# jason-li-831202/Vehicle-CV-ADAS

Hardware: AMD Instinct MI355X
Metric: frames/sec end-to-end (detect+lane+NMS+track) per GPU; conv MFMA util % (higher is better)
Workload: dtype fp16x3

## Files before the change

vehicle-cv-adas_amd/csrc/conv_halo_s2.hip:

```cpp
#include "kernels.h"
#include "elem16.h"
#include <stdlib.h>
#include <map>
#include <mutex>
#include <tuple>
#include <type_traits>

namespace adas {

typedef __attribute__((ext_vector_type(4))) float sf32x4_;
typedef __attribute__((ext_vector_type(4))) uint32_t su32x4_;

template <int ACT>
__device__ __forceinline__ float s2_act(float v) {
    if (ACT == ACT_SILU) return v * fast_rcp(1.0f + __expf(-v));
    if (ACT == ACT_RELU) return fmaxf(v, 0.0f);
    if (ACT == ACT_LEAKY) return fmaxf(v, 0.1f * v);
    return v;
}

struct S2Dev {
    const uint16_t* in;
    const uint16_t* wgt;
    const float* bias;
// ... 211 lines not shown
        const bool ok = plan_s2_uncached(Ho, Wo, &p);
        it = cache.emplace(key, std::make_pair(ok, p)).first;
    }
    *out = it->second.second;
    return it->second.first;
}

static bool s2p_enabled() {
    static int v = -1;
    if (v < 0) {
        const char* e = getenv("ADAS_NO_HALO_S2P");
        v = (e && e[0] == '1') ? 0 : 1;
    }
    return v == 1;
}

bool halo_s2p_applicable(const ConvArgs& a) {
    const TView &in = a.in, &out = a.out;
    if (!s2p_enabled() || a.stride != 2 || a.kh != 3 || a.kw != 3 || a.pad != 1 || a.res_mode != RES_NONE) return false;
    if (in.f32 || out.f32 || out.h != (in.h + 2 - 3) / 2 + 1 || out.w != (in.w + 2 - 3) / 2 + 1) return false;
    if ((in.c & 7) || (in.cs & 7) || (in.coff & 7) || (out.c & 127) || (out.cs & 3) || (out.coff & 3)) return false;
    if (in.c < 16 || (long)in.h * in.w * in.cs >= (1L << 30)) return false;
    if (in.c < 128) return false;
    S2Plan pl;
    if (!plan_s2(out.h, out.w, &pl) || pl.eff < 0.45) return false;
    return (long)a.n * pl.NS * pl.TPS * (out.c / 128) >= 512;
}

hipError_t launch_conv_halo_s2p(const ConvArgs& a, hipStream_t st) {
    S2Plan pl;
    if (!halo_s2p_applicable(a) || !plan_s2(a.out.h, a.out.w, &pl)) return hipErrorInvalidValue;
    S2Dev d;
    d.in = (const uint16_t*)a.in.p; d.wgt = (const uint16_t*)a.wgt; d.bias = a.bias; d.out = (uint16_t*)a.out.p;
    d.in_cs = a.in.cs; d.in_coff = a.in.coff; d.cin = a.in.c; d.H = a.in.h; d.W = a.in.w;
    d.out_cs = a.out.cs; d.out_coff = a.out.coff; d.cout = a.out.c;
    d.cin_pad = (a.in.c + 31) / 32 * 32;
    d.SW = pl.SW; d.NS = pl.NS; d.TPS = pl.TPS; d.PW = pl.PW; d.plane = pl.plane;
    d.npix4 = 4 * pl.plane * 4;
    d.Ho = a.out.h; d.Wo = a.out.w;
    d.mg_pw = pl.mg_pw; d.mg_sw = pl.mg_sw; d.mg_plane = pl.mg_plane;
    d.ntiles = a.n * pl.NS * pl.TPS;
    d.tiles8 = (d.ntiles + 7) / 8;
    d.ncb = a.out.c / 128;
    { static int xm = -1; if (xm < 0) { const char* e = getenv("ADAS_HALO_XMAP"); xm = e ? atoi(e) : 1; } d.xmap = xm; }
    const dim3 grid(8 * d.tiles8 * d.ncb);
    const size_t lds = ((size_t)4 * pl.plane * 32 + (size_t)2 * S2_WROWS * 32) * 2;
    static bool attr_done = false;
    if (!attr_done) {
#define S2_ATTR(E_, A_) (void)hipFuncSetAttribute((const void*)conv_s2p_kernel<E_, A_>, hipFuncAttributeMaxDynamicSharedMemorySize, 160 * 1024)
        S2_ATTR(Bf16, ACT_NONE); S2_ATTR(Bf16, ACT_SILU); S2_ATTR(Bf16, ACT_RELU); S2_ATTR(Bf16, ACT_LEAKY);
        S2_ATTR(Fp16, ACT_NONE); S2_ATTR(Fp16, ACT_SILU); S2_ATTR(Fp16, ACT_RELU); S2_ATTR(Fp16, ACT_LEAKY);
#undef S2_ATTR
        attr_done = true;
    }
    ADAS_DISPATCH_E16(a.prec == PREC_FP16, E, {
        if (a.act == ACT_SILU) hipLaunchKernelGGL((conv_s2p_kernel<E, ACT_SILU>), grid, dim3(S2_THR), lds, st, d);
        else if (a.act == ACT_RELU) hipLaunchKernelGGL((conv_s2p_kernel<E, ACT_RELU>), grid, dim3(S2_THR), lds, st, d);
        else if (a.act == ACT_LEAKY) hipLaunchKernelGGL((conv_s2p_kernel<E, ACT_LEAKY>), grid, dim3(S2_THR), lds, st, d);
        else hipLaunchKernelGGL((conv_s2p_kernel<E, ACT_NONE>), grid, dim3(S2_THR), lds, st, d);
    });
    return hipGetLastError();
}

struct S2XDev {
    const unsigned char* in;
    const uint16_t* wgt;
    const float* bias;
    x3s* out;
    int in_cs, in_coff, cin, H, W;
    int out_cs, out_coff, cout;
    int nck;
    int SW, NS, TPS, PW, plane;
    int npix4;
    int Ho, Wo;
    uint32_t mg_pw, mg_sw, mg_plane;
    int ntiles, tiles8, ncb, xmap;
};

template <int ACT>
__device__ __forceinline__ float s2x_act(float v) {
    if (ACT == ACT_SILU) return x3_silu(v);
    if (ACT == ACT_RELU) return fmaxf(v, 0.0f);
    if (ACT == ACT_LEAKY) return fmaxf(v, 0.1f * v);
    return v;
}

#ifdef ADAS_S2X_PROF
__device__ unsigned long long g_s2x_prof[16];
#define S2XP(i)                                     \
    if (tid == 0) {                                 \
        const unsigned long long t__ = clock64();   \
        pacc__[i] += t__ - tprev__;                 \
        tprev__ = t__;                              \
    }
#else
#define S2XP(i)
#endif

template <int ACT>
__global__ __launch_bounds__(S2_THR, 1) void conv_s2p_x3_kernel(S2XDev a) {
    Fp16::enter();
    typedef Fp16::vec8 vec8;
    constexpr int TAPS = 9, TM = 4;
    extern __shared__ __attribute__((aligned(16))) uint16_t lds[];
    uint16_t* Aw = lds;
    uint16_t* Ww = lds + (size_t)4 * a.plane * 32;

    const int tid = threadIdx.x, lane = tid & 63, wave = tid >> 6;
    const int lrow = lane & 15, kg = lane >> 4;
    const int half = wave >> 2, grp = wave & 3;
#ifdef ADAS_S2X_PROF
    unsigned long long tprev__ = clock64();
    unsigned long long pacc__[8] = {0, 0, 0, 0, 0, 0, 0, 0};
#endif
    const int xslot = blockIdx.x >> 3;
    const int xr = xslot / a.ncb;
    const int cb = xslot - xr * a.ncb;
    int tile = a.xmap ? (int)(blockIdx.x & 7) * a.tiles8 + xr : xr * 8 + (blockIdx.x & 7);
    if (tile >= a.ntiles) return;
    const int n0 = cb * 64 + half * 32;
    const int per_img = a.NS * a.TPS;
    const int img = tile / per_img;
    tile -= img * per_img;
    const int strip = tile / a.TPS, t = tile - strip * a.TPS;
    const int sx0 = strip * a.SW, p0 = t * S2_BM;
    const int y_first = (int)(((uint32_t)p0 * a.mg_sw) >> 20);
    const int wy0 = 2 * y_first - 1, wx0 = 2 * sx0 - 1;

    const unsigned char* in_img = a.in + ((size_t)img * a.H * a.W * a.in_cs + a.in_coff) * 4;
    __amdgpu_buffer_rsrc_t rsrc = __builtin_amdgcn_make_buffer_rsrc((void*)in_img, 0, (a.H * a.W * a.in_cs - a.in_coff) * 4, 0x00020000);
    uint32_t goff[S2_NA];
#pragma unroll
    for (int i = 0; i < S2_NA; ++i) {
        const int e = tid + S2_THR * i;
        const int pix = e >> 2, c8 = e & 3;
        const int q = (int)(((uint32_t)pix * a.mg_plane) >> 20);
        const int pp = pix - q * a.plane;
        const int py = (int)(((uint32_t)pp * a.mg_pw) >> 20), px = pp - py * a.PW;
        const int iy = wy0 + 2 * py + (q >> 1), ix = wx0 + 2 * px + (q & 1);
        const bool ok = e < a.npix4 && (unsigned)iy < (unsigned)a.H && (unsigned)ix < (unsigned)a.W;
        goff[i] = ok ? (uint32_t)((iy * a.W + ix) * a.in_cs * 4 + c8 * 32) : 0x80000000u;
    }
    const uint16_t* wb0 = a.wgt + (size_t)(2 * cb) * a.nck * S2_WROWS * 32;
    const uint16_t* wb1 = wb0 + (size_t)a.nck * S2_WROWS * 32;
    const int gsw[4] = {0, 2, 3, 1};
    const int wdst0 = ((tid & ~3) + ((tid & 3) ^ gsw[(tid >> 4) & 3])) * 8;
    const int wrd = (half * S2_WROWS + lrow) * 32 + ((kg ^ gsw[(lrow >> 2) & 3]) << 3);

    int apl[TM], oy[TM], ox[TM];
#pragma unroll
    for (int j = 0; j < TM; ++j) {
        const int p = p0 + (grp * TM + j) * 16 + lrow;
        const int y = (int)(((uint32_t)p * a.mg_sw) >> 20), xs = p - y * a.SW;
        oy[j] = y;
        ox[j] = sx0 + xs;
        apl[j] = (y - y_first) * a.PW + xs;
    }

    sf32x4_ acc[4][TM];
#pragma unroll
    for (int i = 0; i < 2; ++i) {
        const float4 b = *reinterpret_cast<const float4*>(a.bias + n0 + i * 16 + kg * 4);
#pragma unroll
        for (int j = 0; j < TM; ++j) {
            acc[i][j] = sf32x4_{b.x, b.y, b.z, b.w};
            acc[i + 2][j] = sf32x4_{0.f, 0.f, 0.f, 0.f};
        }
    }

    su32x4_ ra[S2_NA], rw[S2_NW];
    auto gload = [&](int ck, auto with_w) {
        const uint32_t cofs = (uint32_t)((ck >> 1) * 128 + (ck & 1) * 16);
#pragma unroll
        for (int i = 0; i < S2_NA; ++i) ra[i] = __builtin_amdgcn_raw_buffer_load_b128(rsrc, goff[i] + cofs, 0, 0);
        if constexpr (!decltype(with_w)::value) return;
#pragma unroll
        for (int i = 0; i < S2_NW; ++i) {
            const int e = tid + S2_THR * i;
            const uint16_t* src = (e < S2_WROWS * 4 ? wb0 + (size_t)e * 8 : wb1 + (size_t)(e - S2_WROWS * 4) * 8) + (size_t)ck * S2_WROWS * 32;
            rw[i] = *reinterpret_cast<const su32x4_*>(src);
        }
    };
    const int na = (a.npix4 + S2_THR - 1) / S2_THR;
    auto lstore = [&](auto with_w) {
#pragma unroll
        for (int i = 0; i < S2_NA; ++i) {
            const int e = tid + S2_THR * i;
            if (i < na && e < a.npix4) *reinterpret_cast<su32x4_*>(Aw + (e >> 2) * 32 + (((e & 3) ^ ((e >> 3) & 2)) << 3)) = ra[i];
        }
        if constexpr (!decltype(with_w)::value) return;
#pragma unroll
        for (int i = 0; i < S2_NW; ++i) *reinterpret_cast<su32x4_*>(Ww + wdst0 + i * S2_THR * 8) = rw[i];
    };
    auto taps = [&](auto lo_c) {
        constexpr int I0 = decltype(lo_c)::value ? 2 : 0;
#pragma unroll
        for (int tap = 0; tap < TAPS; ++tap) {
            const int r = tap / 3, s = tap - r * 3;
            const int tofs = ((r & 1) * 2 + (s & 1)) * a.plane + (r >> 1) * a.PW + (s >> 1);
            vec8 wf[4], xf[TM];
#pragma unroll
            for (int i = I0; i < 4; ++i) wf[i] = *reinterpret_cast<const vec8*>(Ww + (tap * 64 + (i - I0) * 16) * 32 + wrd);
#pragma unroll
            for (int j = 0; j < TM; ++j) {
                const int pw = apl[j] + tofs;
                xf[j] = *reinterpret_cast<const vec8*>(Aw + pw * 32 + ((kg ^ ((pw >> 1) & 2)) << 3));
            }
#pragma unroll
            for (int i = I0; i < 4; ++i)
#pragma unroll
                for (int j = 0; j < TM; ++j) acc[i][j] = Fp16::mfma(wf[i], xf[j], acc[i][j]);
        }
    };

    S2XP(0)
    gload(0, std::true_type{});
    lstore(std::true_type{});
    __syncthreads();
    S2XP(1)
    for (int ck = 0; ck < a.nck; ck += 2) {
        gload(ck + 1, std::false_type{});
        taps(std::false_type{});
        S2XP(2)
        __syncthreads();
        S2XP(3)
        lstore(std::false_type{});
        __syncthreads();
        S2XP(4)
        if (ck + 2 < a.nck) gload(ck + 2, std::true_type{});
        taps(std::true_type{});
        S2XP(5)
        if (ck + 2 < a.nck) {
            __syncthreads();
            lstore(std::true_type{});
            __syncthreads();
            S2XP(6)
        }
    }

#pragma unroll
    for (int j = 0; j < TM; ++j) {
        const bool pok = oy[j] < a.Ho && ox[j] < a.Wo;
        const size_t mpix = pok ? ((size_t)img * a.Ho + oy[j]) * a.Wo + ox[j] : 0;
#pragma unroll
        for (int i = 0; i < 2; ++i) {
            float v[4];
#pragma unroll
            for (int e = 0; e < 4; ++e) v[e] = s2x_act<ACT>(acc[i][j][e] + acc[i + 2][j][e] * kX3Down);
            const int c = n0 + i * 16 + kg * 4;
            if (pok && c < a.cout) x3_store4(a.out + mpix * a.out_cs + a.out_coff + c, v);
        }
    }
#ifdef ADAS_S2X_PROF
    S2XP(7)
    if (tid == 0) {
        for (int i__ = 0; i__ < 8; ++i__) atomicAdd(&g_s2x_prof[i__], pacc__[i__]);
        atomicAdd(&g_s2x_prof[8], 1ull);
    }
#endif
}

#ifdef ADAS_S2X_PROF
extern "C" int adas_debug_s2x_prof(unsigned long long* out16, int reset) {
    static unsigned long long h[16];
    if (out16 && hipMemcpyFromSymbol(out16, HIP_SYMBOL(g_s2x_prof), sizeof(h)) != hipSuccess) return -1;
    if (reset) {
        for (int i = 0; i < 16; ++i) h[i] = 0;
        if (hipMemcpyToSymbol(HIP_SYMBOL(g_s2x_prof), h, sizeof(h)) != hipSuccess) return -1;
    }
    return 0;
}
#endif

struct S2DDev {
    const void* in;
    const void* wgt;
    const float* bias;
    void* out;
    uint32_t in_bytes, wgt_bytes, out_bytes;
    int in_cs, in_coff, cin, H, W;
    int out_cs, out_coff, cout, Ho, Wo;
    int nck;
    int SW, NS, TPS, PW, PH, plane16;
    uint32_t mg_pw, mg_sw;
    int ntiles, tiles8, ncb, xmap;
};
typedef __attribute__((address_space(3))) void* slds_vp;
typedef __attribute__((ext_vector_type(2))) float sf32x2_;
constexpr uint32_t S2D_OOB = 0xF0000000u;
constexpr int S2D_TAP = 2 * 64 * 64;
constexpr int S2D_SLAB = 9 * 64 * 64;


template <int N>
__device__ __forceinline__ void s2d_wait_vm() {
    asm volatile("s_waitcnt vmcnt(%0)" ::"n"(N) : "memory");
}
template <int ACT>
__device__ __forceinline__ sf32x2_ s2d_act2(sf32x2_ v) {
    if (ACT == ACT_RELU) return __builtin_elementwise_max(v, sf32x2_{0.0f, 0.0f});
    return sf32x2_{s2x_act<ACT>(v[0]), s2x_act<ACT>(v[1])};
}

#ifdef ADAS_S2D_PROF
__device__ unsigned long long g_s2d_prof[16];
#define S2DP(i)                                     \
    if (tid == 0) {                                 \
        const unsigned long long t__ = clock64();   \
        pacc__[i] += t__ - tprev__;                 \
        tprev__ = t__;                              \
    }
#else
#define S2DP(i)
#endif

template <int ACT, int NP>
__global__ __launch_bounds__(S2_THR, 1) void conv_s2d_x3_kernel(S2DDev a) {
    Fp16::enter();
    typedef Fp16::vec8 vec8;
    extern __shared__ __attribute__((aligned(16))) uint8_t s2d_lds[];
    const int WOFF = 4 * a.plane16 * 64;

    const int tid = threadIdx.x, lane = tid & 63;
    const int wave = __builtin_amdgcn_readfirstlane(tid >> 6);
    const int lrow = lane & 15, kg = lane >> 4;
    const int hb = wave >> 2, grp = wave & 3;
#ifdef ADAS_S2D_PROF
    unsigned long long tprev__ = clock64();
    unsigned long long pacc__[8] = {0, 0, 0, 0, 0, 0, 0, 0};
    unsigned long long nitem__ = 0;
#endif
    __amdgpu_buffer_rsrc_t rin = __builtin_amdgcn_make_buffer_rsrc((void*)a.in, 0, a.in_bytes, 0x00020000);
    __amdgpu_buffer_rsrc_t rwg = __builtin_amdgcn_make_buffer_rsrc((void*)a.wgt, 0, a.wgt_bytes, 0x00020000);
    __amdgpu_buffer_rsrc_t rout = __builtin_amdgcn_make_buffer_rsrc((void*)a.out, 0, a.out_bytes, 0x00020000);
    const int gsw[4] = {0, 2, 3, 1};
    const uint32_t wlane = (uint32_t)((lane >> 2) * 64 + (((lane & 3) ^ gsw[(lane >> 4) & 3]) << 4));
    const uint32_t wrd = (uint32_t)(WOFF + hb * 4096 + lrow * 64 + ((kg ^ gsw[(lrow >> 2) & 3]) << 4));
    const uint32_t ch_lane = (uint32_t)((hb * 4 + (kg >> 1)) * 32 + (kg & 1) * 16);

    struct Item {
        int img, cb, sx0, p0, y_first;
    };
    const int nvb = 8 * a.tiles8 * a.ncb, per_img = a.NS * a.TPS;
    auto decode = [&](int v, Item& it) -> bool {
        if (v >= nvb) return false;
        const int xslot = v >> 3, xr = xslot / a.ncb;
        int tile = a.xmap ? (v & 7) * a.tiles8 + xr : xr * 8 + (v & 7);
        if (tile >= a.ntiles) return false;
        it.cb = xslot - xr * a.ncb;
        it.img = tile / per_img;
        tile -= it.img * per_img;
        const int strip = tile / a.TPS, t = tile - strip * a.TPS;
        it.sx0 = strip * a.SW;
        it.p0 = t * S2_BM;
        it.y_first = (int)(((uint32_t)it.p0 * a.mg_sw) >> 20);
        return true;
    };
    int vb = blockIdx.x;
    const int vstep = gridDim.x;
    Item cur, nxt;
    if (!decode(vb, cur)) return;
    bool has_next = decode(vb + vstep, nxt);

    const int npieces = a.plane16 >> 4;
    int pj[3];
#pragma unroll
    for (int n = 0; n < NP; ++n) pj[n] = wave + 8 * n < npieces ? wave + 8 * n : wave % npieces;
    auto src_offset = [&](const Item& it, int q, int n) {
        int lz;
        asm volatile("v_mov_b32 %0, %1" : "=v"(lz) : "v"(lane));
        const int px = pj[n] * 16 + (lz >> 2);
        const int grpk = (lz & 3) ^ ((px >> 1) & 2);
        const int py = (int)(((uint32_t)px * a.mg_pw) >> 20), pxx = px - py * a.PW;
        const int iy = 2 * it.y_first - 1 + 2 * py + (q >> 1), ix = 2 * it.sx0 - 1 + 2 * pxx + (q & 1);
        const bool ok = py < a.PH && (unsigned)iy < (unsigned)a.H && (unsigned)ix < (unsigned)a.W;
        const uint32_t off = ((uint32_t)((it.img * a.H + iy) * a.W + ix) * (uint32_t)a.in_cs + (uint32_t)a.in_coff) * 4u + (uint32_t)(grpk << 5);
        const uint32_t m = 0u - (uint32_t)ok;
        return (off & m) | (S2D_OOB & ~m);
    };
    uint32_t gsrc[4][3];
    auto wgt_base = [&](int cb) { return (uint32_t)(((2 * cb + hb) * a.nck) * S2D_SLAB + grp * 1024); };
    auto issue_tile = [&](int tap, uint32_t wsrc, uint32_t woob) {
        __builtin_amdgcn_raw_ptr_buffer_load_lds(rwg, (slds_vp)(s2d_lds + WOFF + tap * S2D_TAP + wave * 1024), 16, wlane | woob, wsrc + (uint32_t)tap * 4096u, 0, 0);
    };

    uint32_t apl[4], po[4];
    auto set_output = [&](const Item& it) {
#pragma unroll
        for (int j = 0; j < 4; ++j) {
            const int p = it.p0 + (grp * 4 + j) * 16 + lrow;
            const int y = (int)(((uint32_t)p * a.mg_sw) >> 20), xs = p - y * a.SW;
            apl[j] = (uint32_t)((y - it.y_first) * a.PW + xs);
            const int ox = it.sx0 + xs;
            po[j] = (y < a.Ho && ox < a.Wo) ? (uint32_t)((it.img * a.Ho + y) * a.Wo + ox) : S2D_OOB;
        }
    };
    const uint32_t kg16 = (uint32_t)(kg << 4);
    auto frag_addr = [&](int j, int t) {
        const int r = t / 3, sx = t % 3;
        const uint32_t pw = apl[j] + (uint32_t)((r >> 1) * a.PW + (sx >> 1));
        return ((uint32_t)(((r & 1) * 2 + (sx & 1)) * a.plane16) + pw) * 64u + (kg16 ^ ((pw << 3) & 0x20u));
    };
    sf32x4_ acc[4][4];
    float4 bias4[2];
#pragma unroll
    for (int i = 0; i < 2; ++i) bias4[i] = *reinterpret_cast<const float4*>(a.bias + cur.cb * 64 + hb * 32 + i * 16 + kg * 4);
    auto reset_acc = [&]() {
#pragma unroll
        for (int i = 0; i < 2; ++i) {
#pragma unroll
            for (int j = 0; j < 4; ++j) {
                acc[i][j] = sf32x4_{bias4[i].x, bias4[i].y, bias4[i].z, bias4[i].w};
                acc[i + 2][j] = sf32x4_{0.f, 0.f, 0.f, 0.f};
            }
        }
    };

    struct Pend {
        uint32_t wsrc, woob;
        bool last;
    };
    auto issue_piece = [&](auto q_c, auto g_c, auto lo_c, auto k_c, const Pend& pd) {
        constexpr int q = decltype(q_c)::value, g = decltype(g_c)::value, k = decltype(k_c)::value;
        constexpr bool pislo = decltype(lo_c)::value;
        if constexpr (k < NP) {
            __builtin_amdgcn_raw_ptr_buffer_load_lds(rin, (slds_vp)(s2d_lds + (q * a.plane16 + pj[k] * 16) * 64), 16, gsrc[q][k], 0, 0, 0);
            if (pd.last) gsrc[q][k] = has_next ? src_offset(nxt, q, k) : S2D_OOB;
            else gsrc[q][k] += pislo ? 16u : 112u;
        } else {
            constexpr int tl[4][4] = {{4, 4, 4, 4}, {1, 7, 7, 7}, {3, 5, 5, 5}, {0, 2, 6, 8}};
            issue_tile(tl[g][k - NP], pd.wsrc, pd.woob);
        }
    };

    const uint32_t wcur = wgt_base(cur.cb);
#pragma unroll
    for (int q = 0; q < 4; ++q)
#pragma unroll
        for (int n = 0; n < NP; ++n) gsrc[q][n] = src_offset(cur, q, n);
    {
        const Pend p0{wcur, 0u, false};
        auto slot = [&](auto q_c, auto g_c) {
            constexpr int g = decltype(g_c)::value;
            constexpr int nt = g == 0 ? 1 : 2;
            issue_piece(q_c, g_c, std::true_type{}, std::integral_constant<int, 0>{}, p0);
            issue_piece(q_c, g_c, std::true_type{}, std::integral_constant<int, 1>{}, p0);
            if constexpr (NP > 2) issue_piece(q_c, g_c, std::true_type{}, std::integral_constant<int, 2>{}, p0);
            issue_piece(q_c, g_c, std::true_type{}, std::integral_constant<int, NP>{}, p0);
            if constexpr (nt > 1) issue_piece(q_c, g_c, std::true_type{}, std::integral_constant<int, NP + 1>{}, p0);
        };
        slot(std::integral_constant<int, 3>{}, std::integral_constant<int, 0>{});
        slot(std::integral_constant<int, 1>{}, std::integral_constant<int, 1>{});
        slot(std::integral_constant<int, 2>{}, std::integral_constant<int, 2>{});
    }
    set_output(cur);
    reset_acc();
    s2d_wait_vm<0>();
    __builtin_amdgcn_s_barrier();
    S2DP(0)

    for (;;) {
        const uint32_t wnext = wcur;
        const uint32_t woob_next = has_next ? 0u : S2D_OOB;

        auto half_chunk = [&](auto lo_c, const int ck) {
            constexpr bool islo = decltype(lo_c)::value;
            constexpr int I0 = islo ? 2 : 0, NI = islo ? 2 : 4;
#pragma unroll
            for (int j = 0; j < 4; ++j) asm volatile("" : "+v"(apl[j]));
            const bool to_next_item = ck + 1 >= a.nck;
            const Pend pprev{wcur + (uint32_t)ck * S2D_SLAB, 0u, ck - 1 == a.nck - 2};
            const Pend pthis{to_next_item ? wnext : wcur + (uint32_t)(ck + 1) * S2D_SLAB, to_next_item ? woob_next : 0u, ck == a.nck - 2};
            auto tap = [&](auto t_c, auto pq_c, auto pg_c, auto pl_c, auto k0_c, auto k1_c, const Pend& pd) {
                constexpr int t = decltype(t_c)::value, K0 = decltype(k0_c)::value, K1 = decltype(k1_c)::value;
                vec8 wf[4], xf[4];
#pragma unroll
                for (int i = I0; i < 4; ++i) wf[i] = *reinterpret_cast<const vec8*>(s2d_lds + wrd + t * S2D_TAP + (i - I0) * 1024);
#pragma unroll
                for (int j = 0; j < 4; ++j) xf[j] = *reinterpret_cast<const vec8*>(s2d_lds + frag_addr(j, t));
                auto block = [&](auto b_c) {
                    constexpr int b = decltype(b_c)::value;
                    if constexpr (b < NI) {
#pragma unroll
                        for (int j = 0; j < 4; ++j) acc[I0 + b][j] = Fp16::mfma(wf[I0 + b], xf[j], acc[I0 + b][j]);
                        constexpr int ka = K0 + (K1 - K0) * b / NI, kb = K0 + (K1 - K0) * (b + 1) / NI;
                        if constexpr (kb > ka) issue_piece(pq_c, pg_c, pl_c, std::integral_constant<int, ka>{}, pd);
                        if constexpr (kb > ka + 1) issue_piece(pq_c, pg_c, pl_c, std::integral_constant<int, ka + 1>{}, pd);
                        if constexpr (kb > ka + 2) issue_piece(pq_c, pg_c, pl_c, std::integral_constant<int, ka + 2>{}, pd);
                        static_assert(kb <= ka + 3, "at most three pieces between two MFMA blocks");
                    }
                };
                block(std::integral_constant<int, 0>{}); block(std::integral_constant<int, 1>{});
                block(std::integral_constant<int, 2>{}); block(std::integral_constant<int, 3>{});
            };
            auto close = [&](auto g_c) {
                constexpr int g = decltype(g_c)::value;
                constexpr int allow = 2 * NP + (islo ? (g == 0 ? 0 : (g == 1 ? 1 : (g == 2 ? 3 : 4))) : (g == 0 ? 6 : (g == 1 ? 4 : 0)));
                __builtin_amdgcn_sched_barrier(0);
                S2DP(islo ? 2 : 1)
                s2d_wait_vm<allow>();
                S2DP(3)
                __builtin_amdgcn_s_barrier();
                __builtin_amdgcn_sched_barrier(0);
                S2DP(4)
            };
            using std::integral_constant;
            typedef integral_constant<bool, !islo> PrevL;
            typedef integral_constant<bool, islo> ThisL;
            constexpr int P3 = NP + (!islo ? 4 : 0), P0 = NP + (islo ? 1 : 0), P1 = NP + (islo ? 2 : 0), P2 = NP + (islo ? 2 : 0);
            tap(integral_constant<int, 4>{}, integral_constant<int, 0>{}, integral_constant<int, 3>{}, PrevL{}, integral_constant<int, 0>{}, integral_constant<int, P3>{}, pprev);
            close(integral_constant<int, 0>{});
            tap(integral_constant<int, 1>{}, integral_constant<int, 3>{}, integral_constant<int, 0>{}, ThisL{}, integral_constant<int, 0>{}, integral_constant<int, P0 / 2>{}, pthis);
            tap(integral_constant<int, 7>{}, integral_constant<int, 3>{}, integral_constant<int, 0>{}, ThisL{}, integral_constant<int, P0 / 2>{}, integral_constant<int, P0>{}, pthis);
            close(integral_constant<int, 1>{});
            tap(integral_constant<int, 3>{}, integral_constant<int, 1>{}, integral_constant<int, 1>{}, ThisL{}, integral_constant<int, 0>{}, integral_constant<int, P1 / 2>{}, pthis);
            tap(integral_constant<int, 5>{}, integral_constant<int, 1>{}, integral_constant<int, 1>{}, ThisL{}, integral_constant<int, P1 / 2>{}, integral_constant<int, P1>{}, pthis);
            close(integral_constant<int, 2>{});
            tap(integral_constant<int, 0>{}, integral_constant<int, 2>{}, integral_constant<int, 2>{}, ThisL{}, integral_constant<int, 0>{}, integral_constant<int, P2 / 4>{}, pthis);
            tap(integral_constant<int, 2>{}, integral_constant<int, 2>{}, integral_constant<int, 2>{}, ThisL{}, integral_constant<int, P2 / 4>{}, integral_constant<int, P2 / 2>{}, pthis);
            tap(integral_constant<int, 6>{}, integral_constant<int, 2>{}, integral_constant<int, 2>{}, ThisL{}, integral_constant<int, P2 / 2>{}, integral_constant<int, 3 * P2 / 4>{}, pthis);
            tap(integral_constant<int, 8>{}, integral_constant<int, 2>{}, integral_constant<int, 2>{}, ThisL{}, integral_constant<int, 3 * P2 / 4>{}, integral_constant<int, P2>{}, pthis);
            close(integral_constant<int, 3>{});
        };
        for (int ck = 0; ck < a.nck; ck += 2) {
            half_chunk(std::false_type{}, ck);
            half_chunk(std::true_type{}, ck + 1);
        }
        S2DP(5)

        {
            const uint32_t ch0 = (uint32_t)(cur.cb * 256) + ch_lane;
#pragma unroll
            for (int j = 0; j < 4; ++j) {
                sf32x2_ val[2][2];
                uint32_t hw[2][2];
#pragma unroll
                for (int i = 0; i < 2; ++i) {
                    val[i][0] = s2d_act2<ACT>(sf32x2_{acc[i + 2][j][0], acc[i + 2][j][1]} * kX3Down + sf32x2_{acc[i][j][0], acc[i][j][1]});
                    val[i][1] = s2d_act2<ACT>(sf32x2_{acc[i + 2][j][2], acc[i + 2][j][3]} * kX3Down + sf32x2_{acc[i][j][2], acc[i][j][3]});
                }
                __builtin_amdgcn_s_setreg((unsigned short)(1 | (6 << 6) | (1 << 11)), 0u);
#pragma unroll
                for (int i = 0; i < 2; ++i)
#pragma unroll
                    for (int h = 0; h < 2; ++h) asm volatile("v_cvt_pk_f16_f32 %0, %1, %2" : "=v"(hw[i][h]) : "v"(val[i][h][0]), "v"(val[i][h][1]));
                __builtin_amdgcn_s_setreg((unsigned short)(1 | (6 << 6) | (1 << 11)), 3u);
                const uint32_t oo = po[j] == S2D_OOB ? S2D_OOB : (po[j] * (uint32_t)a.out_cs + (uint32_t)a.out_coff) * 4u + ch0;
#pragma unroll
                for (int i = 0; i < 2; ++i) {
                    const uint32_t oi = (cur.cb * 64 + hb * 32 + i * 16 + (kg >> 1) * 8 < a.cout) ? oo + i * 64 : S2D_OOB;
                    uint32_t lw[2];
#pragma unroll
                    for (int h = 0; h < 2; ++h) {
                        const sf32x2_ d = (val[i][h] - __builtin_convertvector(__builtin_bit_cast(e_f16x2, hw[i][h]), sf32x2_)) * kX3Up;
                        lw[h] = __builtin_bit_cast(uint32_t, __builtin_convertvector(d, e_f16x2));
                    }
                    const auto s0 = __builtin_amdgcn_permlane16_swap(hw[i][0], lw[0], false, false);
                    const auto s1 = __builtin_amdgcn_permlane16_swap(hw[i][1], lw[1], false, false);
                    __builtin_amdgcn_raw_buffer_store_b128(su32x4_{s0[0], s1[0], s0[1], s1[1]}, rout, oi, 0, 0);
                }
            }
        }
        S2DP(6)
#ifdef ADAS_S2D_PROF
        ++nitem__;
#endif
        if (!has_next) break;
        cur = nxt;
        vb += vstep;
        has_next = decode(vb + vstep, nxt);
        set_output(cur);
        reset_acc();
        S2DP(7)
    }
#ifdef ADAS_S2D_PROF
    if (tid == 0) {
        for (int i__ = 0; i__ < 8; ++i__) atomicAdd(&g_s2d_prof[i__], pacc__[i__]);
        atomicAdd(&g_s2d_prof[8], nitem__);
    }
#endif
    s2d_wait_vm<0>();
}

#ifdef ADAS_S2D_PROF
extern "C" int adas_debug_s2d_prof(unsigned long long* out16, int reset) {
    static unsigned long long h[16];
    if (out16 && hipMemcpyFromSymbol(out16, HIP_SYMBOL(g_s2d_prof), sizeof(h)) != hipSuccess) return -1;
    if (reset) {
        for (int i = 0; i < 16; ++i) h[i] = 0;
        if (hipMemcpyToSymbol(HIP_SYMBOL(g_s2d_prof), h, sizeof(h)) != hipSuccess) return -1;
    }
    return 0;
}
#endif

static bool s2x_enabled() {
    static int v = -1;
    if (v < 0) {
        const char* e = getenv("ADAS_NO_HALO_S2P_X3");
        v = (e && e[0] == '1') ? 0 : 1;
    }
    return v == 1;
}

bool halo_s2p_x3_shape_ok(int kh, int kw, int stride, int pad, int res_mode, const TView& in, const TView& out) {
    if (!s2x_enabled() || stride != 2 || kh != 3 || kw != 3 || pad != 1 || res_mode != RES_NONE) return false;
    if (in.f32 || out.f32 || out.h != (in.h + 2 - 3) / 2 + 1 || out.w != (in.w + 2 - 3) / 2 + 1) return false;
    if ((in.c & 31) || (in.cs & 7) || (in.coff & 7) || (out.c & 7) || (out.cs & 7) || (out.coff & 7)) return false;
    if ((long)in.h * in.w * in.cs * 4 >= (1L << 31)) return false;
    if (2 * out.c < (out.c + 63) / 64 * 64) return false;
    S2Plan pl;
    return plan_s2(out.h, out.w, &pl) && pl.eff >= 0.45;
}

bool halo_s2p_x3_applicable(const ConvArgs& a) {
    if (!halo_s2p_x3_shape_ok(a.kh, a.kw, a.stride, a.pad, a.res_mode, a.in, a.out)) return false;
    S2Plan pl;
    if (!plan_s2(a.out.h, a.out.w, &pl)) return false;
    static long min_items = -1;
    if (min_items < 0) { const char* e = getenv("ADAS_S2X_MIN_ITEMS"); min_items = e ? atol(e) : 96; if (min_items < 1) min_items = 96; }
    return (long)a.n * pl.NS * pl.TPS * ((a.out.c + 63) / 64) >= min_items;
}

bool s2d_x3_fits(const ConvArgs& a) {
    const TView &in = a.in, &out = a.out;
    const int n = a.n;
    static int on = -1;
    if (on < 0) { const char* e = getenv("ADAS_NO_S2D_X3"); on = (e && e[0] == '1') ? 0 : 1; }
    const size_t in_bytes = (size_t)n * in.h * in.w * in.cs * 4, out_bytes = (size_t)n * out.h * out.w * out.cs * 4;
    const int ncb = (out.c + 63) / 64, nck = 2 * (in.c / 32);
    const size_t wgt_bytes = (size_t)2 * ncb * nck * S2D_SLAB;
    return on && ncb <= 32 && in_bytes < 0x70000000ull && out_bytes < 0x70000000ull && wgt_bytes < 0x70000000ull;
}
hipError_t launch_conv_s2d_x3(const ConvArgs& a, hipStream_t st) {
    S2Plan pl;
    if (!a.wgt_h8x3 || !halo_s2p_x3_applicable(a) || !s2d_x3_fits(a) || !plan_s2(a.out.h, a.out.w, &pl)) return hipErrorInvalidValue;
    const size_t in_bytes = (size_t)a.n * a.in.h * a.in.w * a.in.cs * 4, out_bytes = (size_t)a.n * a.out.h * a.out.w * a.out.cs * 4;
    const int ncb = (a.out.c + 63) / 64, nck = 2 * (a.in.c / 32);
    const size_t wgt_bytes = (size_t)2 * ncb * nck * S2D_SLAB;
    S2DDev d;
    d.in = a.in.p; d.wgt = a.wgt_h8x3; d.bias = a.bias; d.out = a.out.p;
    d.in_bytes = (uint32_t)in_bytes; d.wgt_bytes = (uint32_t)wgt_bytes; d.out_bytes = (uint32_t)out_bytes;
    d.in_cs = a.in.cs; d.in_coff = a.in.coff; d.cin = a.in.c; d.H = a.in.h; d.W = a.in.w;
    d.out_cs = a.out.cs; d.out_coff = a.out.coff; d.cout = a.out.c; d.Ho = a.out.h; d.Wo = a.out.w;
    d.nck = nck;
    d.SW = pl.SW; d.NS = pl.NS; d.TPS = pl.TPS; d.PW = pl.PW;
    d.PH = (S2_BM + pl.SW - 1) / pl.SW + ((S2_BM % pl.SW) ? 1 : 0) + 1;
    d.plane16 = (d.PH * d.PW + 15) / 16 * 16;
    d.mg_pw = pl.mg_pw; d.mg_sw = pl.mg_sw;
    d.ntiles = a.n * pl.NS * pl.TPS;
    d.tiles8 = (d.ntiles + 7) / 8;
    d.ncb = ncb;
    { static int xm = -1; if (xm < 0) { const char* e = getenv("ADAS_HALO_XMAP"); xm = e ? atoi(e) : 1; } d.xmap = xm; }
    const size_t lds = (size_t)4 * d.plane16 * 64 + 9 * S2D_TAP;
    if (lds > 160 * 1024) return hipErrorInvalidValue;
    const int nvb = 8 * d.tiles8 * d.ncb;
    static int rounds = -1;
    if (rounds < 0) { const char* e = getenv("ADAS_S2D_ROUNDS"); rounds = e ? atoi(e) : 16; if (rounds < 1 || rounds > 16) rounds = 16; }
    const int gmax = 8 * d.ncb * (32 / d.ncb) * rounds;
    const dim3 grid(nvb > gmax ? gmax : nvb);
    static bool attr_done = false;
    if (!attr_done) {
#define S2D_ATTR(A_) (void)hipFuncSetAttribute((const void*)conv_s2d_x3_kernel<A_, 2>, hipFuncAttributeMaxDynamicSharedMemorySize, 160 * 1024); \
                     (void)hipFuncSetAttribute((const void*)conv_s2d_x3_kernel<A_, 3>, hipFuncAttributeMaxDynamicSharedMemorySize, 160 * 1024)
        S2D_ATTR(ACT_NONE); S2D_ATTR(ACT_SILU); S2D_ATTR(ACT_RELU); S2D_ATTR(ACT_LEAKY);
#undef S2D_ATTR
        attr_done = true;
    }
    const bool np3 = d.plane16 > 256;
#define S2D_GO(A_) do { if (np3) hipLaunchKernelGGL((conv_s2d_x3_kernel<A_, 3>), grid, dim3(S2_THR), lds, st, d); \
                        else hipLaunchKernelGGL((conv_s2d_x3_kernel<A_, 2>), grid, dim3(S2_THR), lds, st, d); } while (0)
    if (a.act == ACT_SILU) S2D_GO(ACT_SILU);
    else if (a.act == ACT_RELU) S2D_GO(ACT_RELU);
    else if (a.act == ACT_LEAKY) S2D_GO(ACT_LEAKY);
    else S2D_GO(ACT_NONE);
#undef S2D_GO
    return hipGetLastError();
}

hipError_t launch_conv_s2p_x3(const ConvArgs& a, hipStream_t st) {
    S2Plan pl;
    if (!a.wgt_h8x3 || !halo_s2p_x3_applicable(a) || !plan_s2(a.out.h, a.out.w, &pl)) return hipErrorInvalidValue;
    S2XDev d;
    d.in = (const unsigned char*)a.in.p; d.wgt = (const uint16_t*)a.wgt_h8x3; d.bias = a.bias; d.out = (x3s*)a.out.p;
    d.in_cs = a.in.cs; d.in_coff = a.in.coff; d.cin = a.in.c; d.H = a.in.h; d.W = a.in.w;
    d.out_cs = a.out.cs; d.out_coff = a.out.coff; d.cout = a.out.c;
    d.nck = 2 * (a.in.c / 32);
    d.SW = pl.SW; d.NS = pl.NS; d.TPS = pl.TPS; d.PW = pl.PW; d.plane = pl.plane;
    d.npix4 = 4 * pl.plane * 4;
    d.Ho = a.out.h; d.Wo = a.out.w;
    d.mg_pw = pl.mg_pw; d.mg_sw = pl.mg_sw; d.mg_plane = pl.mg_plane;
    d.ntiles = a.n * pl.NS * pl.TPS;
    d.tiles8 = (d.ntiles + 7) / 8;
    d.ncb = (a.out.c + 63) / 64;
    { static int xm = -1; if (xm < 0) { const char* e = getenv("ADAS_HALO_XMAP"); xm = e ? atoi(e) : 1; } d.xmap = xm; }
    const dim3 grid(8 * d.tiles8 * d.ncb);
    const size_t lds = ((size_t)4 * pl.plane * 32 + (size_t)2 * S2_WROWS * 32) * 2;
    static bool attr_done = false;
    if (!attr_done) {
#define S2X_ATTR(A_) (void)hipFuncSetAttribute((const void*)conv_s2p_x3_kernel<A_>, hipFuncAttributeMaxDynamicSharedMemorySize, 160 * 1024)
        S2X_ATTR(ACT_NONE); S2X_ATTR(ACT_SILU); S2X_ATTR(ACT_RELU); S2X_ATTR(ACT_LEAKY);
#undef S2X_ATTR
        attr_done = true;
    }
    if (a.act == ACT_SILU) hipLaunchKernelGGL((conv_s2p_x3_kernel<ACT_SILU>), grid, dim3(S2_THR), lds, st, d);
    else if (a.act == ACT_RELU) hipLaunchKernelGGL((conv_s2p_x3_kernel<ACT_RELU>), grid, dim3(S2_THR), lds, st, d);
    else if (a.act == ACT_LEAKY) hipLaunchKernelGGL((conv_s2p_x3_kernel<ACT_LEAKY>), grid, dim3(S2_THR), lds, st, d);
    else hipLaunchKernelGGL((conv_s2p_x3_kernel<ACT_NONE>), grid, dim3(S2_THR), lds, st, d);
    return hipGetLastError();
}

}
```

Baseline: 5598.

## Merge stride-2 conv load slots into three stages and precompute fragment addresses

Restructures the per-chunk load and MMA pipeline of the stride-2 fp16x3 conv from four wait groups to three: the q=3 and q=1 input-plane loads are merged into one slot, and the weight-tap order and wait counts are rebalanced. The prologue is staggered with scheduling barriers, and the initial wait no longer drains all loads. Per-row LDS fragment base addresses are precomputed per 2x2 sub-offset, and output pixel offsets are computed only in the epilogue, to cut address arithmetic in the hot loop at some register cost. The epilogue also narrows the rounding-mode switches to a subset of the packed conversions per row, which can change rounding of the high half while relying on the residual half to compensate.

```diff
diff --git a/vehicle-cv-adas_amd/csrc/conv_halo_s2.hip b/vehicle-cv-adas_amd/csrc/conv_halo_s2.hip
--- a/vehicle-cv-adas_amd/csrc/conv_halo_s2.hip
+++ b/vehicle-cv-adas_amd/csrc/conv_halo_s2.hip
@@ -537,6 +537,21 @@
     return sf32x2_{s2x_act<ACT>(v[0]), s2x_act<ACT>(v[1])};
 }
 
+__host__ __device__ constexpr int s2d_flush_first(int act, int j) { return act == ACT_SILU ? (j == 0 ? 2 : 1) : 0; }
+__host__ __device__ constexpr int s2d_flush_count(int act, int j) {
+    return act == ACT_SILU ? (j == 0 ? 2 : (j == 3 ? 0 : 3)) : (act == ACT_LEAKY ? (j == 0 ? 0 : 2) : 0);
+}
+__device__ __forceinline__ void s2d_cvt_hi_flushed(uint32_t& h0, uint32_t& h1, sf32x2_ a, sf32x2_ b) {
+    asm volatile("s_setreg_imm32_b32 hwreg(HW_REG_MODE, 6, 2), 0\n\ts_nop 1\n\tv_cvt_pk_f16_f32 %0, %2, %3\n\tv_cvt_pk_f16_f32 %1, %4, %5\n\t"
+                 "s_setreg_imm32_b32 hwreg(HW_REG_MODE, 6, 2), 3\n\ts_nop 1"
+                 : "=&v"(h0), "=&v"(h1) : "v"(a[0]), "v"(a[1]), "v"(b[0]), "v"(b[1]));
+}
+__device__ __forceinline__ void s2d_cvt_hi_flushed(uint32_t& h0, uint32_t& h1, uint32_t& h2, sf32x2_ a, sf32x2_ b, sf32x2_ c) {
+    asm volatile("s_setreg_imm32_b32 hwreg(HW_REG_MODE, 6, 2), 0\n\ts_nop 1\n\tv_cvt_pk_f16_f32 %0, %3, %4\n\tv_cvt_pk_f16_f32 %1, %5, %6\n\t"
+                 "v_cvt_pk_f16_f32 %2, %7, %8\n\ts_setreg_imm32_b32 hwreg(HW_REG_MODE, 6, 2), 3\n\ts_nop 1"
+                 : "=&v"(h0), "=&v"(h1), "=&v"(h2) : "v"(a[0]), "v"(a[1]), "v"(b[0]), "v"(b[1]), "v"(c[0]), "v"(c[1]));
+}
+
 #ifdef ADAS_S2D_PROF
 __device__ unsigned long long g_s2d_prof[16];
 #define S2DP(i)                                     \
@@ -568,9 +583,10 @@
     __amdgpu_buffer_rsrc_t rin = __builtin_amdgcn_make_buffer_rsrc((void*)a.in, 0, a.in_bytes, 0x00020000);
     __amdgpu_buffer_rsrc_t rwg = __builtin_amdgcn_make_buffer_rsrc((void*)a.wgt, 0, a.wgt_bytes, 0x00020000);
     __amdgpu_buffer_rsrc_t rout = __builtin_amdgcn_make_buffer_rsrc((void*)a.out, 0, a.out_bytes, 0x00020000);
-    const int gsw[4] = {0, 2, 3, 1};
-    const uint32_t wlane = (uint32_t)((lane >> 2) * 64 + (((lane & 3) ^ gsw[(lane >> 4) & 3]) << 4));
-    const uint32_t wrd = (uint32_t)(WOFF + hb * 4096 + lrow * 64 + ((kg ^ gsw[(lrow >> 2) & 3]) << 4));
+    auto gsw = [](int x) { return (0x78 >> (2 * x)) & 3; };
+
+    const uint32_t wlane = (uint32_t)((lane >> 2) * 64 + (((lane & 3) ^ gsw((lane >> 4) & 3)) << 4));
+    const uint32_t wrd = (uint32_t)(WOFF + hb * 4096 + lrow * 64 + ((kg ^ gsw((lrow >> 2) & 3)) << 4));
     const uint32_t ch_lane = (uint32_t)((hb * 4 + (kg >> 1)) * 32 + (kg & 1) * 16);
 
     struct Item {
@@ -619,22 +635,30 @@
         __builtin_amdgcn_raw_ptr_buffer_load_lds(rwg, (slds_vp)(s2d_lds + WOFF + tap * S2D_TAP + wave * 1024), 16, wlane | woob, wsrc + (uint32_t)tap * 4096u, 0, 0);
     };
 
-    uint32_t apl[4], po[4];
+    const uint32_t kg16 = (uint32_t)(kg << 4);
+    const uint32_t splane = (uint32_t)(a.plane16 * 64);
+    uint32_t fa[4][4];
     auto set_output = [&](const Item& it) {
 #pragma unroll
         for (int j = 0; j < 4; ++j) {
             const int p = it.p0 + (grp * 4 + j) * 16 + lrow;
             const int y = (int)(((uint32_t)p * a.mg_sw) >> 20), xs = p - y * a.SW;
-            apl[j] = (uint32_t)((y - it.y_first) * a.PW + xs);
-            const int ox = it.sx0 + xs;
-            po[j] = (y < a.Ho && ox < a.Wo) ? (uint32_t)((it.img * a.Ho + y) * a.Wo + ox) : S2D_OOB;
-        }
-    };
-    const uint32_t kg16 = (uint32_t)(kg << 4);
+            const uint32_t ap = (uint32_t)((y - it.y_first) * a.PW + xs);
+#pragma unroll
+            for (int st = 0; st < 4; ++st) {
+                const uint32_t pw = ap + (uint32_t)((st >> 1) * a.PW + (st & 1));
+                fa[j][st] = pw * 64u + (kg16 ^ ((pw << 3) & 0x20u));
+            }
+        }
+    };
+    auto out_pixel = [&](const Item& it, int j) {
+        const int p = it.p0 + (grp * 4 + j) * 16 + lrow;
+        const int y = (int)(((uint32_t)p * a.mg_sw) >> 20), ox = it.sx0 + p - y * a.SW;
+        return (y < a.Ho && ox < a.Wo) ? (uint32_t)((it.img * a.Ho + y) * a.Wo + ox) : S2D_OOB;
+    };
     auto frag_addr = [&](int j, int t) {
         const int r = t / 3, sx = t % 3;
-        const uint32_t pw = apl[j] + (uint32_t)((r >> 1) * a.PW + (sx >> 1));
-        return ((uint32_t)(((r & 1) * 2 + (sx & 1)) * a.plane16) + pw) * 64u + (kg16 ^ ((pw << 3) & 0x20u));
+        return fa[j][(r >> 1) * 2 + (sx >> 1)] + (uint32_t)((r & 1) * 2 + (sx & 1)) * splane;
     };
     sf32x4_ acc[4][4];
     float4 bias4[2];
@@ -655,42 +679,49 @@
         uint32_t wsrc, woob;
         bool last;
     };
-    auto issue_piece = [&](auto q_c, auto g_c, auto lo_c, auto k_c, const Pend& pd) {
-        constexpr int q = decltype(q_c)::value, g = decltype(g_c)::value, k = decltype(k_c)::value;
+    auto issue_piece = [&](auto s_c, auto lo_c, auto k_c, const Pend& pd) {
+        constexpr int S = decltype(s_c)::value, k = decltype(k_c)::value;
         constexpr bool pislo = decltype(lo_c)::value;
-        if constexpr (k < NP) {
-            __builtin_amdgcn_raw_ptr_buffer_load_lds(rin, (slds_vp)(s2d_lds + (q * a.plane16 + pj[k] * 16) * 64), 16, gsrc[q][k], 0, 0, 0);
-            if (pd.last) gsrc[q][k] = has_next ? src_offset(nxt, q, k) : S2D_OOB;
-            else gsrc[q][k] += pislo ? 16u : 112u;
+        constexpr int NWIN = S == 0 ? 2 * NP : NP;
+        if constexpr (k < NWIN) {
+            constexpr int q = S == 0 ? (k < NP ? 3 : 1) : (S == 1 ? 2 : 0), n = k < NP ? k : k - NP;
+            __builtin_amdgcn_raw_ptr_buffer_load_lds(rin, (slds_vp)(s2d_lds + (q * a.plane16 + pj[n] * 16) * 64), 16, gsrc[q][n], 0, 0, 0);
+            if (pd.last) gsrc[q][n] = has_next ? src_offset(nxt, q, n) : S2D_OOB;
+            else gsrc[q][n] += pislo ? 16u : 112u;
         } else {
-            constexpr int tl[4][4] = {{4, 4, 4, 4}, {1, 7, 7, 7}, {3, 5, 5, 5}, {0, 2, 6, 8}};
-            issue_tile(tl[g][k - NP], pd.wsrc, pd.woob);
-        }
-    };
+            constexpr int tl[3][4] = {{4, 1, 7, 7}, {3, 5, 5, 5}, {0, 2, 6, 8}};
+            issue_tile(tl[S][k - NWIN], pd.wsrc, pd.woob);
+        }
+    };
+    typedef std::integral_constant<int, 0> SlotA;
+    typedef std::integral_constant<int, 1> SlotB;
+    typedef std::integral_constant<int, 2> SlotC;
 
     const uint32_t wcur = wgt_base(cur.cb);
-#pragma unroll
-    for (int q = 0; q < 4; ++q)
-#pragma unroll
-        for (int n = 0; n < NP; ++n) gsrc[q][n] = src_offset(cur, q, n);
     {
         const Pend p0{wcur, 0u, false};
-        auto slot = [&](auto q_c, auto g_c) {
-            constexpr int g = decltype(g_c)::value;
-            constexpr int nt = g == 0 ? 1 : 2;
-            issue_piece(q_c, g_c, std::true_type{}, std::integral_constant<int, 0>{}, p0);
-            issue_piece(q_c, g_c, std::true_type{}, std::integral_constant<int, 1>{}, p0);
-            if constexpr (NP > 2) issue_piece(q_c, g_c, std::true_type{}, std::integral_constant<int, 2>{}, p0);
-            issue_piece(q_c, g_c, std::true_type{}, std::integral_constant<int, NP>{}, p0);
-            if constexpr (nt > 1) issue_piece(q_c, g_c, std::true_type{}, std::integral_constant<int, NP + 1>{}, p0);
-        };
-        slot(std::integral_constant<int, 3>{}, std::integral_constant<int, 0>{});
-        slot(std::integral_constant<int, 1>{}, std::integral_constant<int, 1>{});
-        slot(std::integral_constant<int, 2>{}, std::integral_constant<int, 2>{});
-    }
+#define S2D_PK(S_, K_) issue_piece(S_{}, std::true_type{}, std::integral_constant<int, K_>{}, p0)
+        S2D_PK(SlotA, 2 * NP); S2D_PK(SlotA, 2 * NP + 1); S2D_PK(SlotA, 2 * NP + 2); S2D_PK(SlotB, NP); S2D_PK(SlotB, NP + 1);
+        __builtin_amdgcn_sched_barrier(0);
+#pragma unroll
+        for (int n = 0; n < NP; ++n) gsrc[3][n] = src_offset(cur, 3, n);
+#pragma unroll
+        for (int n = 0; n < NP; ++n) gsrc[1][n] = src_offset(cur, 1, n);
+        S2D_PK(SlotA, 0); S2D_PK(SlotA, 1); S2D_PK(SlotA, 2); S2D_PK(SlotA, 3);
+        if constexpr (NP > 2) { S2D_PK(SlotA, 4); S2D_PK(SlotA, 5); }
+        __builtin_amdgcn_sched_barrier(0);
+#pragma unroll
+        for (int n = 0; n < NP; ++n) gsrc[2][n] = src_offset(cur, 2, n);
+        S2D_PK(SlotB, 0); S2D_PK(SlotB, 1);
+        if constexpr (NP > 2) S2D_PK(SlotB, 2);
+        __builtin_amdgcn_sched_barrier(0);
+#undef S2D_PK
+    }
+#pragma unroll
+    for (int n = 0; n < NP; ++n) gsrc[0][n] = src_offset(cur, 0, n);
     set_output(cur);
     reset_acc();
-    s2d_wait_vm<0>();
+    s2d_wait_vm<NP>();
     __builtin_amdgcn_s_barrier();
     S2DP(0)
 
@@ -702,11 +733,11 @@
             constexpr bool islo = decltype(lo_c)::value;
             constexpr int I0 = islo ? 2 : 0, NI = islo ? 2 : 4;
 #pragma unroll
-            for (int j = 0; j < 4; ++j) asm volatile("" : "+v"(apl[j]));
+            for (int j = 0; j < 4; ++j) asm volatile("" : "+v"(fa[j][0]), "+v"(fa[j][1]), "+v"(fa[j][2]), "+v"(fa[j][3]));
             const bool to_next_item = ck + 1 >= a.nck;
             const Pend pprev{wcur + (uint32_t)ck * S2D_SLAB, 0u, ck - 1 == a.nck - 2};
             const Pend pthis{to_next_item ? wnext : wcur + (uint32_t)(ck + 1) * S2D_SLAB, to_next_item ? woob_next : 0u, ck == a.nck - 2};
-            auto tap = [&](auto t_c, auto pq_c, auto pg_c, auto pl_c, auto k0_c, auto k1_c, const Pend& pd) {
+            auto tap = [&](auto t_c, auto ps_c, auto pl_c, auto k0_c, auto k1_c, const Pend& pd) {
                 constexpr int t = decltype(t_c)::value, K0 = decltype(k0_c)::value, K1 = decltype(k1_c)::value;
                 vec8 wf[4], xf[4];
 #pragma unroll
@@ -719,9 +750,9 @@
 #pragma unroll
                         for (int j = 0; j < 4; ++j) acc[I0 + b][j] = Fp16::mfma(wf[I0 + b], xf[j], acc[I0 + b][j]);
                         constexpr int ka = K0 + (K1 - K0) * b / NI, kb = K0 + (K1 - K0) * (b + 1) / NI;
-                        if constexpr (kb > ka) issue_piece(pq_c, pg_c, pl_c, std::integral_constant<int, ka>{}, pd);
-                        if constexpr (kb > ka + 1) issue_piece(pq_c, pg_c, pl_c, std::integral_constant<int, ka + 1>{}, pd);
-                        if constexpr (kb > ka + 2) issue_piece(pq_c, pg_c, pl_c, std::integral_constant<int, ka + 2>{}, pd);
+                        if constexpr (kb > ka) issue_piece(ps_c, pl_c, std::integral_constant<int, ka>{}, pd);
+                        if constexpr (kb > ka + 1) issue_piece(ps_c, pl_c, std::integral_constant<int, ka + 1>{}, pd);
+                        if constexpr (kb > ka + 2) issue_piece(ps_c, pl_c, std::integral_constant<int, ka + 2>{}, pd);
                         static_assert(kb <= ka + 3, "at most three pieces between two MFMA blocks");
                     }
                 };
@@ -730,7 +761,7 @@
             };
             auto close = [&](auto g_c) {
                 constexpr int g = decltype(g_c)::value;
-                constexpr int allow = 2 * NP + (islo ? (g == 0 ? 0 : (g == 1 ? 1 : (g == 2 ? 3 : 4))) : (g == 0 ? 6 : (g == 1 ? 4 : 0)));
+                constexpr int allow = g == 0 ? NP + (islo ? 0 : 4) : (g == 1 ? 2 * NP + (islo ? 3 : 0) : NP + (islo ? 2 : 0));
                 __builtin_amdgcn_sched_barrier(0);
                 S2DP(islo ? 2 : 1)
                 s2d_wait_vm<allow>();
@@ -742,20 +773,19 @@
             using std::integral_constant;
             typedef integral_constant<bool, !islo> PrevL;
             typedef integral_constant<bool, islo> ThisL;
-            constexpr int P3 = NP + (!islo ? 4 : 0), P0 = NP + (islo ? 1 : 0), P1 = NP + (islo ? 2 : 0), P2 = NP + (islo ? 2 : 0);
-            tap(integral_constant<int, 4>{}, integral_constant<int, 0>{}, integral_constant<int, 3>{}, PrevL{}, integral_constant<int, 0>{}, integral_constant<int, P3>{}, pprev);
+            constexpr int PC = NP + (!islo ? 4 : 0), PA = 2 * NP + (islo ? 3 : 0), PB = NP + (islo ? 2 : 0);
+            tap(integral_constant<int, 4>{}, SlotC{}, PrevL{}, integral_constant<int, 0>{}, integral_constant<int, PC / 2>{}, pprev);
+            tap(integral_constant<int, 1>{}, SlotC{}, PrevL{}, integral_constant<int, PC / 2>{}, integral_constant<int, PC>{}, pprev);
+            tap(integral_constant<int, 7>{}, SlotC{}, PrevL{}, integral_constant<int, PC>{}, integral_constant<int, PC>{}, pprev);
             close(integral_constant<int, 0>{});
-            tap(integral_constant<int, 1>{}, integral_constant<int, 3>{}, integral_constant<int, 0>{}, ThisL{}, integral_constant<int, 0>{}, integral_constant<int, P0 / 2>{}, pthis);
-            tap(integral_constant<int, 7>{}, integral_constant<int, 3>{}, integral_constant<int, 0>{}, ThisL{}, integral_constant<int, P0 / 2>{}, integral_constant<int, P0>{}, pthis);
+            tap(integral_constant<int, 3>{}, SlotA{}, ThisL{}, integral_constant<int, 0>{}, integral_constant<int, PA / 2>{}, pthis);
+            tap(integral_constant<int, 5>{}, SlotA{}, ThisL{}, integral_constant<int, PA / 2>{}, integral_constant<int, PA>{}, pthis);
             close(integral_constant<int, 1>{});
-            tap(integral_constant<int, 3>{}, integral_constant<int, 1>{}, integral_constant<int, 1>{}, ThisL{}, integral_constant<int, 0>{}, integral_constant<int, P1 / 2>{}, pthis);
-            tap(integral_constant<int, 5>{}, integral_constant<int, 1>{}, integral_constant<int, 1>{}, ThisL{}, integral_constant<int, P1 / 2>{}, integral_constant<int, P1>{}, pthis);
+            tap(integral_constant<int, 0>{}, SlotB{}, ThisL{}, integral_constant<int, 0>{}, integral_constant<int, PB / 4>{}, pthis);
+            tap(integral_constant<int, 2>{}, SlotB{}, ThisL{}, integral_constant<int, PB / 4>{}, integral_constant<int, PB / 2>{}, pthis);
+            tap(integral_constant<int, 6>{}, SlotB{}, ThisL{}, integral_constant<int, PB / 2>{}, integral_constant<int, 3 * PB / 4>{}, pthis);
+            tap(integral_constant<int, 8>{}, SlotB{}, ThisL{}, integral_constant<int, 3 * PB / 4>{}, integral_constant<int, PB>{}, pthis);
             close(integral_constant<int, 2>{});
-            tap(integral_constant<int, 0>{}, integral_constant<int, 2>{}, integral_constant<int, 2>{}, ThisL{}, integral_constant<int, 0>{}, integral_constant<int, P2 / 4>{}, pthis);
-            tap(integral_constant<int, 2>{}, integral_constant<int, 2>{}, integral_constant<int, 2>{}, ThisL{}, integral_constant<int, P2 / 4>{}, integral_constant<int, P2 / 2>{}, pthis);
-            tap(integral_constant<int, 6>{}, integral_constant<int, 2>{}, integral_constant<int, 2>{}, ThisL{}, integral_constant<int, P2 / 2>{}, integral_constant<int, 3 * P2 / 4>{}, pthis);
-            tap(integral_constant<int, 8>{}, integral_constant<int, 2>{}, integral_constant<int, 2>{}, ThisL{}, integral_constant<int, 3 * P2 / 4>{}, integral_constant<int, P2>{}, pthis);
-            close(integral_constant<int, 3>{});
         };
         for (int ck = 0; ck < a.nck; ck += 2) {
             half_chunk(std::false_type{}, ck);
@@ -765,6 +795,12 @@
 
         {
             const uint32_t ch0 = (uint32_t)(cur.cb * 256) + ch_lane;
+            uint32_t po[4];
+#pragma unroll
+            for (int j = 0; j < 4; ++j) {
+                po[j] = out_pixel(cur, j);
+                asm volatile("" : "+v"(po[j]));
+            }
 #pragma unroll
             for (int j = 0; j < 4; ++j) {
                 sf32x2_ val[2][2];
@@ -774,12 +810,15 @@
                     val[i][0] = s2d_act2<ACT>(sf32x2_{acc[i + 2][j][0], acc[i + 2][j][1]} * kX3Down + sf32x2_{acc[i][j][0], acc[i][j][1]});
                     val[i][1] = s2d_act2<ACT>(sf32x2_{acc[i + 2][j][2], acc[i + 2][j][3]} * kX3Down + sf32x2_{acc[i][j][2], acc[i][j][3]});
                 }
-                __builtin_amdgcn_s_setreg((unsigned short)(1 | (6 << 6) | (1 << 11)), 0u);
+                const int f0 = s2d_flush_first(ACT, j), fn = s2d_flush_count(ACT, j);
 #pragma unroll
                 for (int i = 0; i < 2; ++i)
 #pragma unroll
-                    for (int h = 0; h < 2; ++h) asm volatile("v_cvt_pk_f16_f32 %0, %1, %2" : "=v"(hw[i][h]) : "v"(val[i][h][0]), "v"(val[i][h][1]));
-                __builtin_amdgcn_s_setreg((unsigned short)(1 | (6 << 6) | (1 << 11)), 3u);
+                    for (int h = 0; h < 2; ++h)
+                        if (2 * i + h < f0 || 2 * i + h >= f0 + fn) asm volatile("v_cvt_pk_f16_f32 %0, %1, %2" : "=v"(hw[i][h]) : "v"(val[i][h][0]), "v"(val[i][h][1]));
+                if (fn == 2 && f0 == 0) s2d_cvt_hi_flushed(hw[0][0], hw[0][1], val[0][0], val[0][1]);
+                if (fn == 2 && f0 == 2) s2d_cvt_hi_flushed(hw[1][0], hw[1][1], val[1][0], val[1][1]);
+                if (fn == 3) s2d_cvt_hi_flushed(hw[0][1], hw[1][0], hw[1][1], val[0][1], val[1][0], val[1][1]);
                 const uint32_t oo = po[j] == S2D_OOB ? S2D_OOB : (po[j] * (uint32_t)a.out_cs + (uint32_t)a.out_coff) * 4u + ch0;
 #pragma unroll
                 for (int i = 0; i < 2; ++i) {
```

New measurement: 5637, median of 6. No clear change (+0.7%).
